# Agricultural-Robotics-Bonn/pagnerf

Hardware: NVIDIA B200
Metric: train rays/s (march+encode+decode+composite+backward) (higher is better)
Workload: dtype fp16 operands / f32 accumulate (decoders, tcgen05) + f32 (encoders, compositing) = the reference's autocast

## Files before the change

pagnerf_b200/csrc/decoder_tc.cu:

```cuda
#include "decoder_tc_common.cuh"

#define DC_THREADS 512
#define DC_NCG 4
#define DC_MAXK 4

struct DcTcLayout {
    int INP, nXc;
    int oG3, oGy, oOnesA, oX, oHd, oOnesB, oCin, oH1, oOnesC, oH2, oWd1, oWd2, oWc1, oWc2, oWc3, oBias, oPF, oDX, oXI, total;
};
__host__ __device__ inline DcTcLayout dc_tc_layout(int IN, bool bwd, bool img = false) {
    DcTcLayout l;
    l.INP = (IN + 15) & ~15;
    l.nXc = l.INP / 8;
    int o = 0;
    l.oG3 = o; o += bwd ? 2 * TCH : 0;
    l.oGy = o; o += bwd ? 2 * TCH : 0;
    l.oOnesA = o; o += bwd ? 2 * TCH : 0;
    l.oX = o; o += 8 * TCH;
    l.oHd = o; o += 8 * TCH;
    l.oOnesB = o; o += bwd ? 2 * TCH : 0;
    l.oCin = o; o += bwd ? 6 * TCH : 0;
    l.oH1 = o; o += bwd ? 8 * TCH : 0;
    l.oOnesC = o; o += bwd ? 2 * TCH : 0;
    l.oH2 = o; o += bwd ? 8 * TCH : 0;
// ... 149 lines not shown
        if (warp == 0 && elect_one()) { tc_fence_after(); mma16_fwd(tm + 64, aT1, wc2, 64, 64, 64, false); mb.commit(); }
        mb.wait();
        epi_relu16(tl + 64 + c16, bias + 144 + c16, T0 + 2 * cg * TCH, row);
        sync_to_mma();
        if (warp == 0 && elect_one()) { tc_fence_after(); mma16_fwd(tm, aT0, wc3, 16, 16, 64, false); mb.commit(); }
        mb.wait();
        if (cg == 0) {
            float c[16];
            tmem_ld16(tl, c);
            if (valid) {
#pragma unroll
                for (int j = 0; j < 3; ++j) rgb[3 * m + j] = 1.f / (1.f + __expf(-(c[j] + bias[208 + j])));
            }
        }
        tc_fence_before();
        __syncthreads();
    }
    tc_fence_before();
    __syncthreads();
    if (warp == 0) tmem_dealloc(tm, 128);
}

#define DCB_S0 0
#define DCB_S1 64
#define DCB_DWD1 128
#define DCB_DWD2 208
#define DCB_DWC1 288
#define DCB_DWC2 352
#define DCB_DWC3 432

struct DcWsLayout { int oWd1, oWd2, oWc1, oWc2, oWc3, total; };
__host__ __device__ inline DcWsLayout dc_ws_layout(int IN) {
    DcWsLayout w;
    int o = 0;
    w.oWd1 = o; o += 64 * IN;
    w.oWd2 = o; o += 16 * 64;
    w.oWc1 = o; o += (64 * CIN + 3) & ~3;
    w.oWc2 = o; o += 64 * 64;
    w.oWc3 = o; o += 3 * 64;
    w.total = o;
    return w;
}

template <bool IMG>
__global__ void __maxnreg__(96) dc_tc_bwd_kernel(const float* __restrict__ feats, const float* __restrict__ lodw,
                                                               const float* __restrict__ ray_d, int S, int64_t M, int IN,
                                                               DcParams p, const float* __restrict__ g_sigma,
                                                               const float* __restrict__ g_rgb, const float* __restrict__ scale_ptr,
                                                               float* __restrict__ g_feats, float* __restrict__ g_dir,
                                                               const int64_t* __restrict__ m_dev, const int64_t* __restrict__ ridx,
                                                               const uint4* __restrict__ pe16, float* __restrict__ ws) {
    if (m_dev) M = min(M, __ldg(m_dev));
    extern __shared__ __align__(128) uint8_t sm[];
    __shared__ uint64_t bar_s;
    __shared__ uint64_t xbar_s[2];
    __shared__ uint32_t tmem_s;
    __shared__ float gdir_s[2][128][3];
    const DcTcLayout l = dc_tc_layout(IN, true, IMG);
    const int tid = threadIdx.x, warp = warp_id_uniform(), lane = tid & 31;
    const int q = warp & 3, cg = warp >> 2, row = 32 * q + lane, c16 = 16 * cg;
    dc_tc_stage(sm, l, p, IN, lodw);
    for (int i = tid; i < 3 * 2 * TCH / 16; i += DC_THREADS) {
        const int t = i / (2 * TCH / 16), j = i - t * (2 * TCH / 16);
        uint4 u = make_uint4(0u, 0u, 0u, 0u);
        if (j < TCH / 16) u.x = 0x00003C00u;
        reinterpret_cast<uint4*>(sm + (t == 0 ? l.oOnesA : (t == 1 ? l.oOnesB : l.oOnesC)))[j] = u;
        if (IMG && t < 2) reinterpret_cast<uint4*>(sm + l.oXI + t * (2 + l.nXc) * TCH)[j] = u;
    }
    if (tid == 0) { mbar_init(&bar_s, 1); mbar_init(&xbar_s[0], 1); mbar_init(&xbar_s[1], 1); fence_mbar_init(); }
    if (warp == 0) tmem_alloc(&tmem_s, 512);
    sync_to_mma();
    tc_fence_after();
    const uint32_t tm = tmem_s, tl = tm + ((uint32_t)(q * 32) << 16);
    MmaBar mb{&bar_s, 0};
    const float* bias = reinterpret_cast<const float*>(sm + l.oBias);
    uint8_t *G3 = sm + l.oG3, *Gy = sm + l.oGy, *X = sm + l.oX, *Cin = sm + l.oCin, *Hd = sm + l.oHd, *H1 = sm + l.oH1, *H2 = sm + l.oH2;
    const uint32_t aG3 = smem_u32(G3), aGy = smem_u32(Gy), aX = smem_u32(X), aCin = smem_u32(Cin), aHd = smem_u32(Hd),
                   aH1 = smem_u32(H1), aH2 = smem_u32(H2), aOnesA = smem_u32(sm + l.oOnesA), aOnesB = smem_u32(sm + l.oOnesB),
                   aOnesC = smem_u32(sm + l.oOnesC);
    const uint32_t wd1 = smem_u32(sm + l.oWd1), wd2 = smem_u32(sm + l.oWd2), wc1 = smem_u32(sm + l.oWc1),
                   wc2 = smem_u32(sm + l.oWc2), wc3 = smem_u32(sm + l.oWc3);
    float4* pf = reinterpret_cast<float4*>(sm + l.oPF);
    const float scale = scale_ptr ? __ldg(scale_ptr) : 1.f;
    const float inv_scale = 1.f / scale;
    const bool do_rgb = g_rgb != nullptr;
    const int64_t ntiles = (M + 127) / 128;
    const uint32_t xbytes = (uint32_t)l.nXc * TCH, xstride = (uint32_t)(2 + l.nXc) * TCH;
    const uint8_t* fimg = reinterpret_cast<const uint8_t*>(feats);
    uint32_t xpar = 0;
    int xb = 0;
    if (IMG) {
        if ((int64_t)blockIdx.x < ntiles && warp == 0 && elect_one()) {
            mbar_expect_tx(&xbar_s[0], xbytes);
            bulk_g2s(sm + l.oXI + 2 * TCH, fimg + (size_t)blockIdx.x * xbytes, xbytes, &xbar_s[0]);
        }
    } else {
        if ((int64_t)blockIdx.x < ntiles) xpfc_issue<DC_MAXK>(pf, feats, nullptr, IN, (int64_t)blockIdx.x * 128, M);
        cp_async_wait_all();
    }
    __syncthreads();
    bool first = true;
    float* dxs = reinterpret_cast<float*>(sm + l.oDX);
    int64_t dx_tile = -1;
    for (int64_t tile = blockIdx.x; tile < ntiles; tile += gridDim.x, first = false, xb ^= 1) {
        const int64_t m = tile * 128 + row;
        const bool valid = m < M;
        const int64_t mm = valid ? m : M - 1;
        const uint32_t aXt = IMG ? smem_u32(sm + l.oXI + xb * xstride + 2 * TCH) : aX;
        const uint32_t aOnesXt = IMG ? smem_u32(sm + l.oXI + xb * xstride) : aOnesA;
        if (IMG) {
            if (g_feats && dx_tile >= 0 && warp == 0 && elect_one()) bulk_wait_read_all();
            if (tile + gridDim.x < ntiles && warp == 0 && elect_one()) {
                mbar_expect_tx(&xbar_s[xb ^ 1], xbytes);
                bulk_g2s(sm + l.oXI + (xb ^ 1) * xstride + 2 * TCH, fimg + (size_t)(tile + gridDim.x) * xbytes, xbytes, &xbar_s[xb ^ 1]);
            }
            mbar_wait(&xbar_s[xb], (xpar >> xb) & 1u);
            xpar ^= 1u << xb;
        } else {
            if (g_feats && dx_tile >= 0) dx_copy_out(dxs, g_feats, IN, dx_tile * 128, M);
            xpfc_consume<DC_NCG, DC_MAXK>(pf, false, IN, l.INP, X, row, cg);
        }
        float gs_row = 0.f, gr0 = 0.f, gr1 = 0.f, gr2 = 0.f;
        uint4 pa = make_uint4(0u, 0u, 0u, 0u), pb = pa;
        int64_t r = 0;
        if (cg == 0) {
            if (g_sigma && valid) gs_row = __ldg(g_sigma + m);
            if (do_rgb && valid) { gr0 = __ldg(g_rgb + 3 * m); gr1 = __ldg(g_rgb + 3 * m + 1); gr2 = __ldg(g_rgb + 3 * m + 2); }
        } else if (do_rgb && cg <= 2) {
            r = ridx ? ridx[mm] : mm / S;
            if (pe16) { pa = __ldg(pe16 + r * 4 + 2 * (cg - 1)); pb = __ldg(pe16 + r * 4 + 2 * (cg - 1) + 1); }
        }
        sync_to_mma();
        if (warp == 0 && elect_one()) { tc_fence_after(); mma16_fwd(tm + DCB_S0, aXt, wd1, 64, 64, l.INP, false); mb.commit(); }
        if (!IMG && tile + gridDim.x < ntiles)
            xpfc_issue<DC_MAXK>(pf, feats, nullptr, IN, (tile + gridDim.x) * 128, M);
        mb.wait();
        const uint32_t mask_d = epi_relu16(tl + DCB_S0 + c16, bias + c16, Hd + 2 * cg * TCH, row);
        sync_to_mma();
        if (warp == 0 && elect_one()) { tc_fence_after(); mma16_fwd(tm + DCB_S1, aHd, wd2, 16, 16, 64, false); mb.commit(); }
        mb.wait();
        bool y0pos = false;
        float vdir[3] = {0.f, 0.f, 0.f};
        uint32_t mask_1 = 0, mask_2 = 0;
        float dy[16];
#pragma unroll
        for (int i = 0; i < 16; ++i) dy[i] = 0.f;
        if (cg == 0) {
            float y[16];
            tmem_ld16(tl + DCB_S1, y);
#pragma unroll
            for (int i = 0; i < 16; ++i) y[i] += bias[64 + i];
            y0pos = y[0] > 0.f;
            if (do_rgb) { tile_store8(Cin, 0, row, y); tile_store8(Cin, 1, row, y + 8); }
        } else if (do_rgb && cg <= 2) {
            if (pe16 && !g_dir) stage_cin_pe16(Cin, row, cg, pa, pb);
            else {
                vdir[0] = -ray_d[3 * r]; vdir[1] = -ray_d[3 * r + 1]; vdir[2] = -ray_d[3 * r + 2];
                stage_cin_pe(Cin, row, cg, -vdir[0], -vdir[1], -vdir[2]);
            }
        }
        if (do_rgb) {
            sync_to_mma();
            if (warp == 0 && elect_one()) { tc_fence_after(); mma16_fwd(tm + DCB_S0, aCin, wc1, 64, 64, 48, false); mb.commit(); }
            mb.wait();
            mask_1 = epi_relu16(tl + DCB_S0 + c16, bias + 80 + c16, H1 + 2 * cg * TCH, row);
            sync_to_mma();
            if (warp == 0 && elect_one()) { tc_fence_after(); mma16_fwd(tm + DCB_S1, aH1, wc2, 64, 64, 64, false); mb.commit(); }
            mb.wait();
            mask_2 = epi_relu16(tl + DCB_S1 + c16, bias + 144 + c16, H2 + 2 * cg * TCH, row);
            sync_to_mma();
            if (warp == 0 && elect_one()) { tc_fence_after(); mma16_fwd(tm + DCB_S0, aH2, wc3, 16, 16, 64, false); mb.commit(); }
            mb.wait();
            if (cg == 0) {
                float c[16], g[16];
                tmem_ld16(tl + DCB_S0, c);
#pragma unroll
                for (int j = 0; j < 16; ++j) g[j] = 0.f;
                if (valid) {
                    const float gr[3] = {gr0, gr1, gr2};
#pragma unroll
                    for (int j = 0; j < 3; ++j) {
                        const float sg = 1.f / (1.f + __expf(-(c[j] + bias[208 + j])));
                        g[j] = gr[j] * sg * (1.f - sg) * scale;
                    }
                }
                tile_store8(G3, 0, row, g); tile_store8(G3, 1, row, g + 8);
            }
            sync_to_mma();
            if (warp == 0 && elect_one()) {
                tc_fence_after();
                mma16_bwd_weight(tm + DCB_DWC3, aG3, aOnesC, 80, !first);
                mma16_bwd_data(tm + DCB_S1, aG3, wc3, 64, 16, 16, false);
                mb.commit();
            }
            mb.wait();
            epi_grad16_nb(tl + DCB_S1 + c16, mask_2, H2 + 2 * cg * TCH, row);
            sync_to_mma();
            if (warp == 0 && elect_one()) {
                tc_fence_after();
                mma16_bwd_weight(tm + DCB_DWC2, aH2, aH1, 80, !first);
                mma16_bwd_data(tm + DCB_S0, aH2, wc2, 64, 64, 64, false);
                mb.commit();
            }
            mb.wait();
            epi_grad16_nb(tl + DCB_S0 + c16, mask_1, H1 + 2 * cg * TCH, row);
            sync_to_mma();
            if (warp == 0 && elect_one()) {
                tc_fence_after();
                mma16_bwd_weight(tm + DCB_DWC1, aH1, aOnesB, 64, !first);
                mma16_bwd_data(tm + DCB_S1, aH1, wc1, 48, 64, 64, false);
                mb.commit();
            }
            mb.wait();
            if (cg == 0) {
                tmem_ld16(tl + DCB_S1, dy);
            } else if (cg <= 2 && g_dir) {
                float g[16];
                tmem_ld16(tl + DCB_S1 + c16, g);
                float gv[3] = {0.f, 0.f, 0.f};
#pragma unroll
                for (int i = 0; i < 16; ++i) {
                    const int k = 16 * (cg - 1) + i;
                    if (k < 3) gv[k] += g[i];
                    else if (k < 3 + 3 * PE_F) { const int f = (k - 3) / 3, c = (k - 3) % 3; const float b = (float)(1 << f); gv[c] += b * cosf(vdir[c] * b) * g[i]; }
                    else if (k < PE_DIM) { const int f = (k - 3 - 3 * PE_F) / 3, c = (k - 3 - 3 * PE_F) % 3; const float b = (float)(1 << f); gv[c] -= b * sinf(vdir[c] * b) * g[i]; }
                }
                gdir_s[cg - 1][row][0] = gv[0]; gdir_s[cg - 1][row][1] = gv[1]; gdir_s[cg - 1][row][2] = gv[2];
            }
            if (g_dir) {
                __syncthreads();
                if (cg == 0 && valid) {
#pragma unroll
                    for (int c = 0; c < 3; ++c) g_dir[3 * m + c] = -(gdir_s[0][row][c] + gdir_s[1][row][c]) * inv_scale;
                }
            }
        } else if (g_dir && valid && cg == 0) {
            g_dir[3 * m] = 0.f; g_dir[3 * m + 1] = 0.f; g_dir[3 * m + 2] = 0.f;
        }
        if (cg == 0) {
            if (y0pos) dy[0] += gs_row * scale;
            if (!valid) {
#pragma unroll
                for (int i = 0; i < 16; ++i) dy[i] = 0.f;
            }
            tile_store8(Gy, 0, row, dy); tile_store8(Gy, 1, row, dy + 8);
        }
        sync_to_mma();
        if (warp == 0 && elect_one()) {
            tc_fence_after();
            mma16_bwd_weight(tm + DCB_DWD2, aGy, aHd, 80, !first);
            mma16_bwd_data(tm + DCB_S0, aGy, wd2, 64, 16, 16, false);
            mb.commit();
        }
        mb.wait();
        epi_grad16_nb(tl + DCB_S0 + c16, mask_d, Hd + 2 * cg * TCH, row);
        sync_to_mma();
        if (warp == 0 && elect_one()) {
            tc_fence_after();
            mma16_bwd_weight(tm + DCB_DWD1, aHd, aOnesXt, 16 + l.INP, !first);
            if (g_feats) mma16_bwd_data(tm + DCB_S1, aHd, wd1, l.INP, 64, 64, false);
            mb.commit();
        }
        mb.wait();
        if (IMG) {
            if (g_feats && c16 < l.INP) {
                float v[16];
                tmem_ld16(tl + DCB_S1 + c16, v);
                tile_store8(sm + l.oDX, 2 * cg, row, v);
                tile_store8(sm + l.oDX, 2 * cg + 1, row, v + 8);
                fence_async_smem();
            }
            dx_tile = tile;
            tc_fence_before();
            __syncthreads();
            if (g_feats && warp == 0 && elect_one()) bulk_s2g(reinterpret_cast<uint8_t*>(g_feats) + (size_t)tile * xbytes, sm + l.oDX, xbytes);
        } else {
            if (g_feats && c16 < l.INP) dx_stage16(tl + DCB_S1, dxs, row, IN, c16, inv_scale);
            dx_tile = tile;
            cp_async_wait_all();
            tc_fence_before();
            __syncthreads();
        }
    }
    if (IMG) {
        if (g_feats && dx_tile >= 0 && warp == 0 && elect_one()) bulk_wait_read_all();
    } else if (g_feats && dx_tile >= 0) dx_copy_out(dxs, g_feats, IN, dx_tile * 128, M);
    if (!first) {
        tc_fence_after();
        const bool plain = ws != nullptr;
        const DcWsLayout wl = dc_ws_layout(IN);
        float* wsb = plain ? ws + (size_t)blockIdx.x * wl.total : nullptr;
        float *dWd1 = plain ? wsb + wl.oWd1 : p.gWd1, *dWd2 = plain ? wsb + wl.oWd2 : p.gWd2, *dWc1 = plain ? wsb + wl.oWc1 : p.gWc1,
              *dWc2 = plain ? wsb + wl.oWc2 : p.gWc2, *dWc3 = plain ? wsb + wl.oWc3 : p.gWc3;
        if (c16 < l.INP) {
            float v[16];
            tmem_ld16(tl + DCB_DWD1 + 16 + c16, v);
            if (row < 64) {
#pragma unroll
                for (int i = 0; i < 16; ++i)
                    if (c16 + i < IN) {
                        const float x = v[i] * inv_scale * (lodw ? __ldg(lodw + c16 + i) : 1.f);
                        float* d = dWd1 + (size_t)row * IN + c16 + i;
                        if (plain) *d = x; else red_add_f32(d, x);
                    }
            }
        }
        flush_dw16(tl + DCB_DWD2, dWd2, row, 16, 64, c16, inv_scale, plain);
        if (do_rgb) {
            if (c16 < 48) flush_dw16(tl + DCB_DWC1 + 16, dWc1, row, 64, CIN, c16, inv_scale, plain);
            flush_dw16(tl + DCB_DWC2, dWc2, row, 64, 64, c16, inv_scale, plain);
            flush_dw16(tl + DCB_DWC3 + 16, dWc3, row, 3, 64, c16, inv_scale, plain);
        }
        if (cg == 0) {
            float v[16];
            tmem_ld16(tl + DCB_DWD1, v);
            if (row < 64) red_add_f32(p.gbd1 + row, v[0] * inv_scale);
            tmem_ld16(tl + DCB_DWD2 + 64, v);
            if (row < 16) red_add_f32(p.gbd2 + row, v[0] * inv_scale);
            if (do_rgb) {
                tmem_ld16(tl + DCB_DWC1, v);
                if (row < 64) red_add_f32(p.gbc1 + row, v[0] * inv_scale);
                tmem_ld16(tl + DCB_DWC2 + 64, v);
                if (row < 64) red_add_f32(p.gbc2 + row, v[0] * inv_scale);
                tmem_ld16(tl + DCB_DWC3, v);
                if (row < 3) red_add_f32(p.gbc3 + row, v[0] * inv_scale);
            }
        }
    }
    tc_fence_before();
    __syncthreads();
    if (warp == 0) tmem_dealloc(tm, 512);
// ... 491 lines not shown
```

pagnerf_b200/csrc/decoder_tc_common.cuh:

```cuda
#pragma once
#include "decoder_common.cuh"
#include "tc_common.cuh"
#include <cuda_fp16.h>

#define TCH TC_CHUNK_BYTES

#ifdef PAG_PHASE_TIMING
static __device__ unsigned long long pag_phase_clk[64];
#define PAG_PHASE_READER(name)                                                                        \
    extern "C" int name(unsigned long long* host64, int reset) {                                      \
        cudaError_t e = cudaMemcpyFromSymbol(host64, pag_phase_clk, sizeof(unsigned long long) * 64); \
        if (e != cudaSuccess) return (int)e;                                                          \
        if (reset) {                                                                                  \
            unsigned long long z[64] = {0};                                                           \
            e = cudaMemcpyToSymbol(pag_phase_clk, z, sizeof(z));                                      \
        }                                                                                             \
        return (int)e;                                                                                \
    }
#define PAG_PHASE_INIT()                                                     \
    __shared__ unsigned long long _ph_s[64];                                 \
    if (threadIdx.x < 64) _ph_s[threadIdx.x] = 0ull;                         \
    __syncthreads();                                                         \
    unsigned long long _ph_t = clock64()
#define PAG_PHASE(i)                                                         \
// ... 77 lines not shown
            const float send = hi ? v[i] : v[i + n];
            const float keep = hi ? v[i + n] : v[i];
            v[i] = keep + __shfl_xor_sync(0xffffffffu, send, o);
        }
    }
}
__device__ __forceinline__ int scatter_base(int lane, int n) {
    int f = 0, h = n / 2;
    for (int o = 16; o >= 1; o >>= 1, h >>= 1) f += (lane & o) ? h : 0;
    return f;
}
__device__ __forceinline__ void epi_grad64(uint32_t taddr, uint64_t mask, uint8_t* tile, int row, int lane, float (&dbacc)[2]) {
    float g[64];
#pragma unroll
    for (int c0 = 0; c0 < 64; c0 += 16) {
        float v[16];
        tmem_ld16(taddr + c0, v);
#pragma unroll
        for (int i = 0; i < 16; ++i) g[c0 + i] = ((mask >> (c0 + i)) & 1ull) ? v[i] : 0.f;
        tile_store8(tile, c0 / 8, row, g + c0);
        tile_store8(tile, c0 / 8 + 1, row, g + c0 + 8);
    }
    warp_reduce_scatter<64>(g, lane);
    dbacc[0] += g[0]; dbacc[1] += g[1];
}
__device__ __forceinline__ void grad16_store(float (&g)[16], uint8_t* tile, int row, int lane, float& dbacc) {
    tile_store8(tile, 0, row, g);
    tile_store8(tile, 1, row, g + 8);
#pragma unroll
    for (int o = 16, n = 8; o >= 2; o >>= 1, n >>= 1) {
        const bool hi = lane & o;
#pragma unroll
        for (int i = 0; i < n; ++i) {
            const float send = hi ? g[i] : g[i + n];
            const float keep = hi ? g[i + n] : g[i];
            g[i] = keep + __shfl_xor_sync(0xffffffffu, send, o);
        }
    }
    dbacc += g[0] + __shfl_xor_sync(0xffffffffu, g[0], 1);
}
__device__ __forceinline__ uint32_t epi_relu16(uint32_t taddr, const float* __restrict__ bias, uint8_t* tile2, int row) {
    float v[16];
    tmem_ld16(taddr, v);
    uint32_t mask = 0;
#pragma unroll
    for (int i = 0; i < 16; ++i) {
        v[i] = fmaxf(v[i] + bias[i], 0.f);
        mask |= (v[i] > 0.f) ? (1u << i) : 0u;
    }
    tile_store8(tile2, 0, row, v);
    tile_store8(tile2, 1, row, v + 8);
    return mask;
}
__device__ __forceinline__ void epi_grad16(uint32_t taddr, uint32_t mask, uint8_t* tile2, int row, int lane, float& dbacc) {
    float v[16];
    tmem_ld16(taddr, v);
#pragma unroll
    for (int i = 0; i < 16; ++i) v[i] = ((mask >> i) & 1u) ? v[i] : 0.f;
    grad16_store(v, tile2, row, lane, dbacc);
}
__device__ __forceinline__ void epi_grad16_nb(uint32_t taddr, uint32_t mask, uint8_t* tile2, int row) {
    float v[16];
    tmem_ld16(taddr, v);
#pragma unroll
    for (int i = 0; i < 16; ++i) v[i] = ((mask >> i) & 1u) ? v[i] : 0.f;
    tile_store8(tile2, 0, row, v);
    tile_store8(tile2, 1, row, v + 8);
}
struct WsSegs { int n; int off[6]; int len[6]; float* dst[6]; };
#define WS_GROUPS 16
static __global__ void __launch_bounds__(256) ws_reduce_kernel(const float* __restrict__ ws, int nblocks, int64_t M, const int64_t* __restrict__ m_dev,
                                                               int total, WsSegs segs) {
    if (m_dev) M = min(M, __ldg(m_dev));
    const int64_t ntiles = (M + 127) / 128;
    const int nact = (int)(ntiles < nblocks ? ntiles : nblocks);
    const int i = blockIdx.x * blockDim.x + threadIdx.x;
    if (i >= total) return;
    float* dst = nullptr;
#pragma unroll
    for (int s = 0; s < 6; ++s)
        if (s < segs.n && i >= segs.off[s] && i < segs.off[s] + segs.len[s] && segs.dst[s]) dst = segs.dst[s] + (i - segs.off[s]);
    if (!dst) return;
    float a0 = 0.f, a1 = 0.f;
    int b = blockIdx.y;
    for (; b + WS_GROUPS < nact; b += 2 * WS_GROUPS) { a0 += ws[(size_t)b * total + i]; a1 += ws[(size_t)(b + WS_GROUPS) * total + i]; }
    if (b < nact) a0 += ws[(size_t)b * total + i];
    if (blockIdx.y < nact) red_add_f32(dst, a0 + a1);
}

__device__ __forceinline__ void flush_dw16(uint32_t taddr, float* __restrict__ gW, int row, int OUT, int IN, int c0, float inv_scale,
                                           bool plain = false) {
    float v[16];
    tmem_ld16(taddr + c0, v);
    if (row < OUT) {
        float* dst = gW + (size_t)row * IN + c0;
        if (!(IN & 3) && !(reinterpret_cast<uintptr_t>(gW) & 15)) {
#pragma unroll
            for (int i = 0; i < 16; i += 4)
                if (c0 + i < IN) {
                    if (plain) *reinterpret_cast<float4*>(dst + i) = make_float4(v[i] * inv_scale, v[i + 1] * inv_scale, v[i + 2] * inv_scale, v[i + 3] * inv_scale);
                    else red_add_f32x4(dst + i, v[i] * inv_scale, v[i + 1] * inv_scale, v[i + 2] * inv_scale, v[i + 3] * inv_scale);
                }
        } else {
#pragma unroll
            for (int i = 0; i < 16; ++i)
                if (c0 + i < IN) {
                    if (plain) dst[i] = v[i] * inv_scale;
                    else red_add_f32(dst + i, v[i] * inv_scale);
                }
        }
    }
}

__device__ __forceinline__ void flush_dw(uint32_t taddr, float* __restrict__ gW, int row, int OUT, int IN, int ncols, float inv_scale) {
    for (int c0 = 0; c0 < ncols; c0 += 16) {
        float v[16];
        tmem_ld16(taddr + c0, v);
        if (row < OUT) {
// ... 214 lines not shown
```

pagnerf_b200/csrc/decoder_tc_fused.cu:

```cuda
#include "decoder_tc_common.cuh"

struct PanCompFwdLayout {
    int INP, nXc, CsP, CiP;
    int oX, oT1, oT2, oStage, oCR, oWs1, oWs2, oWi1, oWi2, oWi3, oBias, total;
};
__host__ __device__ inline PanCompFwdLayout pan_comp_fwd_layout(int IN, int Cs, int Ci) {
    PanCompFwdLayout l;
    l.INP = (IN + 15) & ~15; l.nXc = l.INP / 8;
    l.CsP = 16; l.CiP = Ci > 0 ? ((Ci + 15) & ~15) : 16;
    int o = 0;
    l.oX = o; o += l.nXc * TCH;
    l.oT1 = o; o += 8 * TCH;
    l.oT2 = o; o += 8 * TCH;
    l.oStage = 0;
    l.oCR = o; o += 4 * 32 * 8;
    o = (o + 15) & ~15;
    l.oWs1 = o; o += l.nXc * 64 * 16;
    l.oWs2 = o; o += 8 * l.CsP * 16;
    l.oWi1 = o; o += l.nXc * 64 * 16;
    l.oWi2 = o; o += 8 * 64 * 16;
    l.oWi3 = o; o += 8 * l.CiP * 16;
    l.oBias = o; o += (64 + l.CsP + 64 + 64 + l.CiP) * 4;
    l.total = o;
    return l;
// ... 203 lines not shown
#pragma unroll
                                for (int i = 0; i < 16; ++i) v[i] = fmaf(v[i], s2, bi3[c0 + 16 * h + i]);
                            }
#pragma unroll
                            for (int i = 0; i < 16; i += 2)
                                *reinterpret_cast<__half2*>(stage + lane * STG_LD + 16 * h + i) = __floats2half2_rn(v[i], v[i + 1]);
                        }
                    }
                    __syncwarp();
                    comp_block(stage, wc, wr, bmask, nrows, out_inst, Ci, c0, lane);
                    __syncwarp();
                }
            }
        }
        if (Cs > 0 && cg == 0) {
            float z[16];
            tmem_ld16(tl + semcol, z);
            float mx = -INFINITY, sum = 0.f;
#pragma unroll
            for (int j = 0; j < 16; ++j) { z[j] += bs2[j]; if (j < Cs) mx = fmaxf(mx, z[j]); }
#pragma unroll
            for (int j = 0; j < 16; ++j) { z[j] = (j < Cs) ? (sem_softmax ? __expf(z[j] - mx) : z[j]) : 0.f; sum += z[j]; }
            const float inv = sem_softmax ? 1.f / sum : 1.f;
#pragma unroll
            for (int j = 0; j < 16; ++j) stage[lane * STG_LD + j] = __float2half_rn(z[j] * inv);
            __syncwarp();
            comp_block(stage, wc, wr, bmask, nrows, out_sem, Cs, 0, lane);
            __syncwarp();
        }
        tc_fence_before();
        __syncthreads();
    }
    tc_fence_before();
    __syncthreads();
    if (warp == 0) tmem_dealloc(tm, 256);
}

#define PCB_S0 0
#define PCB_S1 64
#define PCB_SEMLOG 128
#define PCB_DW1J 208
#define PCB_DWS2T 256
#define PCB_DWI2 272
#define PCB_DWI3 352

#define PCB_THREADS 512
#define PCB_NCG 4
#define PCB_MAXK 3
#define PCB_NGC 16
#define PCB_SEM_CG 3

struct PanCompBwdLayout {
    int INP, nXc, CsP, CiP, nGi;
    int oGs, oX, oHs, oH1, oOnes, oH2, oGi, oW1, oWs2, oWi2, oWi3, oBias, oGC, oGSC, oPF, total;
};
__host__ __device__ inline PanCompBwdLayout pan_comp_bwd_layout(int IN, int Cs, int Ci, bool img = false) {
    PanCompBwdLayout l;
    l.INP = (IN + 15) & ~15; l.nXc = l.INP / 8;
    l.CsP = 16; l.CiP = Ci > 0 ? ((Ci + 15) & ~15) : 16; l.nGi = l.CiP / 8;
    int o = 0;
    l.oGs = o; o += 2 * TCH;
    l.oX = o; o += l.nXc * TCH;
    l.oHs = o; o += 8 * TCH;
    l.oH1 = o; o += 8 * TCH;
    l.oOnes = o; o += 2 * TCH;
    l.oH2 = o; o += 8 * TCH;
    l.oGi = o; o += l.nGi * TCH;
    l.oW1 = o; o += l.nXc * 128 * 16;
    l.oWs2 = o; o += 8 * l.CsP * 16;
    l.oWi2 = o; o += 8 * 64 * 16;
    l.oWi3 = o; o += 8 * l.CiP * 16;
    l.oBias = o; o += (64 + l.CsP + 64 + 64 + l.CiP) * 4;
    const int need = l.oGi + (l.nGi > 16 ? 32 : 16) * TCH;
    if (o < need) o = need;
    o = (o + 15) & ~15;
    l.oGC = o; o += PCB_NGC * l.CiP * 2;
    o = (o + 15) & ~15;
    l.oGSC = o; o += img ? PCB_NGC * 16 * 4 : 0;
    o = (o + 127) & ~127;
    l.oPF = o; o += img ? 2 * l.nXc * TCH : 2 * PCB_MAXK * PCB_THREADS * 16;
    l.total = o;
    return l;
}

struct PanWsLayout { int oWs1, oWs2, oWi1, oWi2, oWi3, total; };
__host__ __device__ inline PanWsLayout pan_ws_layout(int IN, int Cs, int Ci) {
    PanWsLayout w;
    int o = 0;
    w.oWs1 = o; o += 64 * IN;
    w.oWs2 = o; o += (Cs * 64 + 3) & ~3;
    w.oWi1 = o; o += 64 * IN;
    w.oWi2 = o; o += 64 * 64;
    w.oWi3 = o; o += (Ci * 64 + 3) & ~3;
    w.total = o;
    return w;
}
__device__ __forceinline__ void stage_w16_part(__half* img, const float* __restrict__ W, int OUT, int IN, int rows, int row0, int OUTP, int INP,
                                               const float* __restrict__ colscale) {
    const int n = (INP / 8) * rows * 8;
    for (int i = threadIdx.x; i < n; i += blockDim.x) {
        const int e = i & 7, r = (i >> 3) % rows, c = (i >> 3) / rows, in = c * 8 + e;
        float v = 0.f;
        if (W && r < OUT && in < IN) { v = __ldg(W + (size_t)r * IN + in); if (colscale) v *= __ldg(colscale + in); }
        img[((size_t)c * OUTP + row0 + r) * 8 + e] = __float2half_rn(v);
    }
}

__device__ __forceinline__ void load_g16(const __half* __restrict__ gc_row, const float* __restrict__ grow, int c0, int C, bool vec4,
                                         float scale, float (&g)[16]) {
    if (gc_row) {
        const uint4 a = *reinterpret_cast<const uint4*>(gc_row + c0), b = *reinterpret_cast<const uint4*>(gc_row + c0 + 8);
        const uint32_t u[8] = {a.x, a.y, a.z, a.w, b.x, b.y, b.z, b.w};
#pragma unroll
        for (int i = 0; i < 8; ++i) {
            const float2 f = __half22float2(*reinterpret_cast<const __half2*>(&u[i]));
            g[2 * i] = f.x; g[2 * i + 1] = f.y;
        }
    } else {
#pragma unroll
        for (int i = 0; i < 16; i += 4) {
            float4 t;
            if (vec4) t = (c0 + i < C) ? __ldg(reinterpret_cast<const float4*>(grow + c0 + i)) : make_float4(0.f, 0.f, 0.f, 0.f);
            else t = make_float4(c0 + i < C ? __ldg(grow + c0 + i) : 0.f, c0 + i + 1 < C ? __ldg(grow + c0 + i + 1) : 0.f,
                                 c0 + i + 2 < C ? __ldg(grow + c0 + i + 2) : 0.f, c0 + i + 3 < C ? __ldg(grow + c0 + i + 3) : 0.f);
            g[i] = __half2float(__float2half_rn(t.x * scale)); g[i + 1] = __half2float(__float2half_rn(t.y * scale));
            g[i + 2] = __half2float(__float2half_rn(t.z * scale)); g[i + 3] = __half2float(__float2half_rn(t.w * scale));
        }
    }
}

template <bool IMG>
__global__ void __launch_bounds__(PCB_THREADS) pan_comp_bwd_kernel(
    const float* __restrict__ feats, const float* __restrict__ dfeats, const float* __restrict__ lodw, int64_t M, int IN,
    PanParams p, int Cs, int Ci, int sem_softmax, int inst_softmax, float inst_inv_temp,
    const float* __restrict__ w, const float* __restrict__ alpha, const int64_t* __restrict__ ridx,
    const float* __restrict__ g_sem, const float* __restrict__ g_inst, int64_t R, const float* __restrict__ inst_lse,
    const float* __restrict__ scale_ptr, float* __restrict__ g_panop, const int64_t* __restrict__ m_dev, float* __restrict__ ws,
    float* __restrict__ gw_sem, float* __restrict__ gw_inst) {
    if (m_dev) M = min(M, __ldg(m_dev));
    extern __shared__ __align__(128) uint8_t sm[];
    __shared__ uint64_t bar_s;
    __shared__ uint64_t xbar_s;
    __shared__ uint32_t tmem_s;
    __shared__ float part_s[PCB_NCG][128];
    const PanCompBwdLayout l = pan_comp_bwd_layout(IN, Cs, Ci, IMG);
    const int tid = threadIdx.x, warp = warp_id_uniform(), lane = tid & 31;
    const int q = warp & 3, cg = warp >> 2;
    const int row = 32 * q + lane;
    const bool do_sem = (Cs > 0) && g_sem, do_inst = (Ci > 0) && g_inst;
    const float s2 = inst_softmax ? inst_inv_temp * LOG2E_F : inst_inv_temp;
    uint8_t *Gs = sm + l.oGs, *X = sm + l.oX, *Hs = sm + l.oHs, *H1 = sm + l.oH1, *H2 = sm + l.oH2, *Gi = sm + l.oGi;
    {
        float* b = reinterpret_cast<float*>(sm + l.oBias);
        __half* w1 = reinterpret_cast<__half*>(sm + l.oW1);
        stage_w16_part(w1, do_sem ? p.Ws1 : nullptr, 64, IN, 64, 0, 128, l.INP, lodw);
        stage_w16_part(w1, do_inst ? p.Wi1 : nullptr, 64, IN, 64, 64, 128, l.INP, lodw);
        if (do_sem) {
            stage_w16(reinterpret_cast<__half*>(sm + l.oWs2), p.Ws2, Cs, 64, l.CsP, 64);
            stage_b32(b, p.bs1, 64, 64); stage_b32(b + 64, p.bs2, Cs, l.CsP);
        }
        if (do_inst) {
            stage_w16(reinterpret_cast<__half*>(sm + l.oWi2), p.Wi2, 64, 64, 64, 64);
            stage_w16(reinterpret_cast<__half*>(sm + l.oWi3), p.Wi3, Ci, 64, l.CiP, 64);
            stage_b32(b + 64 + l.CsP, p.bi1, 64, 64); stage_b32(b + 128 + l.CsP, p.bi2, 64, 64);
            stage_bi3_scaled(b + 192 + l.CsP, p.bi3, Ci, l.CiP, s2, inst_softmax);
        }
        for (int i = tid; i < 2 * TCH / 16; i += PCB_THREADS) {
            uint4 u = make_uint4(0u, 0u, 0u, 0u);
            if (i < TCH / 16) u.x = 0x00003C00u;
            reinterpret_cast<uint4*>(sm + l.oOnes)[i] = u;
        }
        for (int i = tid; i < PCB_NGC * l.CiP / 8; i += PCB_THREADS)
            reinterpret_cast<uint4*>(sm + l.oGC)[i] = make_uint4(0u, 0u, 0u, 0u);
        if (!do_sem) for (int i = tid; i < 8 * TCH / 16; i += PCB_THREADS) reinterpret_cast<uint4*>(Hs)[i] = make_uint4(0u, 0u, 0u, 0u);
        if (!do_inst) for (int i = tid; i < 8 * TCH / 16; i += PCB_THREADS) reinterpret_cast<uint4*>(H1)[i] = make_uint4(0u, 0u, 0u, 0u);
    }
    if (tid == 0) { mbar_init(&bar_s, 1); mbar_init(&xbar_s, 1); fence_mbar_init(); }
    if (warp == 0) tmem_alloc(&tmem_s, 512);
    sync_to_mma();
    tc_fence_after();
    const uint32_t tm = tmem_s, tl = tm + ((uint32_t)(q * 32) << 16);
    MmaBar mb{&bar_s, 0};
    const float* bias = reinterpret_cast<const float*>(sm + l.oBias);
    const float *bs1 = bias, *bs2 = bias + 64, *bi1 = bias + 64 + l.CsP, *bi2 = bi1 + 64, *bi3 = bi2 + 64;
    const uint32_t aGs = smem_u32(Gs), aX = smem_u32(X), aHs = smem_u32(Hs), aH1 = smem_u32(H1), aH2 = smem_u32(H2), aGi = smem_u32(Gi),
                   aOnes = smem_u32(sm + l.oOnes);
    const uint32_t w1j = smem_u32(sm + l.oW1), ws2 = smem_u32(sm + l.oWs2), wi2 = smem_u32(sm + l.oWi2), wi3 = smem_u32(sm + l.oWi3);
    __half* gcache = reinterpret_cast<__half*>(sm + l.oGC);
    float* gsc = reinterpret_cast<float*>(sm + l.oGSC);
    const float scale = scale_ptr ? __ldg(scale_ptr) : 1.f;
    const float inv_scale = 1.f / scale;
    const int c16 = 16 * cg;
    const bool vec4 = !(Ci & 3);
    float db_s1 = 0.f, db_i1 = 0.f, db_s2 = 0.f;
    const int64_t ntiles = (M + 127) / 128;
    float4* pf = reinterpret_cast<float4*>(sm + l.oPF);
    int64_t n_ray = 0, n_ray0 = 0;
    float n_w = 0.f, n_lse = 0.f;
    const uint32_t xbytes = (uint32_t)l.nXc * TCH;
    uint8_t *XL = sm + l.oPF, *DL = sm + l.oPF + xbytes;
    const uint8_t *fimg = reinterpret_cast<const uint8_t*>(feats), *dimg = reinterpret_cast<const uint8_t*>(dfeats);
    uint32_t xpar = 0;
    if ((int64_t)blockIdx.x < ntiles) {
        const int64_t m0 = min((int64_t)blockIdx.x * 128 + row, M - 1);
        if (IMG) {
            if (warp == 0 && elect_one()) {
                mbar_expect_tx(&xbar_s, dimg ? 2 * xbytes : xbytes);
                bulk_g2s(XL, fimg + (size_t)blockIdx.x * xbytes, xbytes, &xbar_s);
                if (dimg) bulk_g2s(DL, dimg + (size_t)blockIdx.x * xbytes, xbytes, &xbar_s);
            }
        } else {
            xpfc_issue<PCB_MAXK>(pf, feats, dfeats, IN, (int64_t)blockIdx.x * 128, M);
        }
        n_ray = ridx[m0]; n_w = __ldg(w + m0); n_ray0 = ridx[(int64_t)blockIdx.x * 128];
        if (inst_lse) n_lse = __ldg(inst_lse + m0);
    }
    const int ci1 = Ci > 0 ? Ci : 1;
    const int gc_r0 = tid / ci1, gc_c0 = tid % ci1, gc_dr = PCB_THREADS / ci1, gc_dc = PCB_THREADS % ci1;
    bool first = true;
    float* dxs = reinterpret_cast<float*>(Hs);
    int64_t dx_tile = -1;
    PAG_PHASE_INIT();
    if (!IMG) cp_async_wait_all();
    __syncthreads();
    for (int64_t tile = blockIdx.x; tile < ntiles; tile += gridDim.x, first = false) {
        const int64_t m = tile * 128 + row;
        const bool valid = m < M;
        const int64_t mm = valid ? m : M - 1;
        const int64_t ray = n_ray, ray0 = n_ray0;
        const float w_row = n_w, lse_row = n_lse;
        const float a_row = __ldg(alpha + ray);
        if (IMG) {
            if (g_panop && dx_tile >= 0 && warp == 0 && elect_one()) bulk_wait_read_all();
            PAG_PHASE(0);
            mbar_wait(&xbar_s, xpar);
            xpar ^= 1u;
            tile_add16(X, XL, dimg ? DL : nullptr, (int)xbytes);
        } else {
            if (g_panop && dx_tile >= 0) dx_copy_out(dxs, g_panop, IN, dx_tile * 128, M);
            PAG_PHASE(0);
            xpfc_consume<PCB_NCG, PCB_MAXK>(pf, dfeats != nullptr, IN, l.INP, X, row, cg);
        }
        PAG_PHASE(1);
        {
            const int64_t tn = tile + gridDim.x;
            if (tn < ntiles) {
                const int64_t mn = min(tn * 128 + row, M - 1);
                n_ray = ridx[mn]; n_w = __ldg(w + mn); n_ray0 = ridx[tn * 128];
                if (inst_lse) n_lse = __ldg(inst_lse + mn);
            }
        }
        sync_to_mma(); PAG_PHASE(2);
        if (warp == 0 && elect_one()) {
            tc_fence_after();
            mma16_fwd(tm + PCB_S0, aX, w1j, 128, 128, l.INP, false);
            mb.commit();
        }
        PAG_PHASE(17);
        if (tile + gridDim.x < ntiles) {
            if (IMG) {
                if (warp == 0 && elect_one()) {
                    mbar_expect_tx(&xbar_s, dimg ? 2 * xbytes : xbytes);
                    bulk_g2s(XL, fimg + (size_t)(tile + gridDim.x) * xbytes, xbytes, &xbar_s);
                    if (dimg) bulk_g2s(DL, dimg + (size_t)(tile + gridDim.x) * xbytes, xbytes, &xbar_s);
                }
            } else {
                xpfc_issue<PCB_MAXK>(pf, feats, dfeats, IN, (tile + gridDim.x) * 128, M);
            }
        }
        PAG_PHASE(18);
        float gpre[7], gspre = 0.f;
        const int ngc_elems = PCB_NGC * Ci;
        if (IMG && do_sem && tid < PCB_NGC * Cs) {
            const int64_t src = ray0 * Cs + tid;
            gspre = (src < R * Cs) ? __ldg(g_sem + src) : 0.f;
        }
        if (do_inst) {
#pragma unroll
            for (int k = 0; k < 7; ++k) {
                const int e = tid + PCB_THREADS * k;
                const int64_t src = ray0 * Ci + e;
                gpre[k] = (e < ngc_elems && src < R * Ci) ? __ldg(g_inst + src) : 0.f;
            }
        }
        PAG_PHASE(19);
        mb.wait(); PAG_PHASE(3);
        const float cs = valid ? a_row * w_row : 0.f;
        uint32_t mask_s = 0, mask_1 = 0, mask_2 = 0;
        if (do_sem) {
// ... 86 lines not shown
                part_s[cg][row] = dot;
                __syncthreads(); PAG_PHASE(8);
                dot = (part_s[0][row] + part_s[1][row]) + (part_s[2][row] + part_s[3][row]);
                if (gw_inst && cg == 0 && valid) gw_inst[m] = dot * inv_scale;
            }
            const float c2 = cs * inst_inv_temp;
#pragma unroll
            for (int k = 0; k < 4; ++k) {
                const int c0 = 16 * (cg + PCB_NCG * k);
                if (c0 < l.CiP) {
                    float v[16], g[16];
                    load_g16(gc_row, grow, c0, Ci, vec4, scale, g);
                    if (inst_softmax) {
                        tmem_ld16(tl + c0, v);
#pragma unroll
                        for (int i = 0; i < 16; ++i) v[i] = c2 * v[i] * (g[i] - dot);
                    } else {
#pragma unroll
                        for (int i = 0; i < 16; ++i) v[i] = c2 * g[i];
                    }
                    tile_store8(Gi + (c0 / 8) * TCH, 0, row, v);
                    tile_store8(Gi + (c0 / 8) * TCH, 1, row, v + 8);
                }
            }
        }
        sync_to_mma(); PAG_PHASE(9);
        if (warp == 0 && elect_one()) {
            tc_fence_after();
            if (do_inst) {
                mma16_bwd_weight(tm + PCB_DWI3, aGi, aOnes, 80, !first);
                if (l.CiP > 128) mma16_bwd_weight(tm + PCB_DWI3 + 80, aGi + 16 * TCH, aOnes, 80, !first);
                mma16_bwd_data(tm + PCB_S1, aGi, wi3, 64, l.CiP, l.CiP, false);
            }
            if (do_sem) {
                mma16_bwd_weight(tm + PCB_DWS2T, aHs, aGs, 16, !first);
                mma16_bwd_data(tm + PCB_S0, aGs, ws2, 64, l.CsP, l.CsP, false);
            }
            mb.commit();
        }
        mb.wait(); PAG_PHASE(10);
        if (do_inst) epi_grad16_nb(tl + PCB_S1 + c16, mask_2, H2 + 2 * cg * TCH, row);
        if (do_sem) epi_grad16(tl + PCB_S0 + c16, mask_s, Hs + 2 * cg * TCH, row, lane, db_s1);
        if (do_inst) {
            sync_to_mma(); PAG_PHASE(11);
            if (warp == 0 && elect_one()) {
                tc_fence_after();
                mma16_bwd_weight(tm + PCB_DWI2, aH2, aH1, 80, !first);
                mma16_bwd_data(tm + PCB_S1, aH2, wi2, 64, 64, 64, false);
                mb.commit();
            }
            mb.wait(); PAG_PHASE(12);
            epi_grad16(tl + PCB_S1 + c16, mask_1, H1 + 2 * cg * TCH, row, lane, db_i1);
        }
        sync_to_mma(); PAG_PHASE(13);
        if (warp == 0 && elect_one()) {
            tc_fence_after();
            mma16_bwd_weight(tm + PCB_DW1J, aHs, aX, l.INP, !first);
            if (g_panop) mma16_bwd_data(tm + PCB_S0, aHs, w1j, l.INP, 128, 128, false);
            mb.commit();
        }
        mb.wait(); PAG_PHASE(14);
        if (IMG) {
            if (g_panop && c16 < l.INP) {
                float v[16];
                tmem_ld16(tl + PCB_S0 + c16, v);
                tile_store8(Hs, 2 * cg, row, v);
                tile_store8(Hs, 2 * cg + 1, row, v + 8);
                fence_async_smem();
            }
            dx_tile = tile;
            tc_fence_before();
            __syncthreads(); PAG_PHASE(15);
            if (g_panop && warp == 0 && elect_one()) bulk_s2g(reinterpret_cast<uint8_t*>(g_panop) + (size_t)tile * xbytes, Hs, xbytes);
        } else {
            if (g_panop && c16 < l.INP) dx_stage16(tl + PCB_S0, dxs, row, IN, c16, inv_scale);
            dx_tile = tile;
            cp_async_wait_all();
            tc_fence_before();
            __syncthreads(); PAG_PHASE(15);
        }
    }
    if (IMG) {
        if (g_panop && dx_tile >= 0 && warp == 0 && elect_one()) bulk_wait_read_all();
    } else if (g_panop && dx_tile >= 0) dx_copy_out(dxs, g_panop, IN, dx_tile * 128, M);
    if (!first) {
        tc_fence_after();
        const int f1 = scatter_base(lane, 32) >> 1;
        const bool own = !(lane & 1);
        const bool plain = ws != nullptr;
        const PanWsLayout wl = pan_ws_layout(IN, Cs, Ci);
        float* wsb = plain ? ws + (size_t)blockIdx.x * wl.total : nullptr;
        float *dWs1 = plain ? wsb + wl.oWs1 : p.gWs1, *dWs2 = plain ? wsb + wl.oWs2 : p.gWs2, *dWi1 = plain ? wsb + wl.oWi1 : p.gWi1,
              *dWi2 = plain ? wsb + wl.oWi2 : p.gWi2, *dWi3 = plain ? wsb + wl.oWi3 : p.gWi3;
        if (c16 < l.INP) {
            float* gW1 = (row < 64) ? (do_sem ? dWs1 : nullptr) : (do_inst ? dWi1 : nullptr);
            float v[16];
            tmem_ld16(tl + PCB_DW1J + c16, v);
            if (gW1) {
#pragma unroll
                for (int i = 0; i < 16; ++i)
                    if (c16 + i < IN) {
                        const float x = v[i] * inv_scale * (lodw ? __ldg(lodw + c16 + i) : 1.f);
                        float* d = gW1 + (size_t)(row & 63) * IN + c16 + i;
                        if (plain) *d = x; else red_add_f32(d, x);
                    }
            }
        }
        if (do_sem) {
            if (cg == 0) {
                float v[16];
                tmem_ld16(tl + PCB_DWS2T, v);
                if (row < 64) {
#pragma unroll
                    for (int j = 0; j < 16; ++j)
                        if (j < Cs) { if (plain) dWs2[(size_t)j * 64 + row] = v[j] * inv_scale; else red_add_f32(dWs2 + (size_t)j * 64 + row, v[j] * inv_scale); }
                }
            }
            if (own) red_add_f32(p.gbs1 + c16 + f1, db_s1 * inv_scale);
            if (own && cg == PCB_SEM_CG && f1 < Cs) red_add_f32(p.gbs2 + f1, db_s2 * inv_scale);
        }
        if (do_inst) {
            flush_dw16(tl + PCB_DWI2, dWi2, row, 64, 64, c16, inv_scale, plain);
            flush_dw16(tl + PCB_DWI3 + 16, dWi3, row, Ci, 64, c16, inv_scale, plain);
            if (l.CiP > 128) flush_dw16(tl + PCB_DWI3 + 96, dWi3 + (size_t)128 * 64, row, Ci - 128, 64, c16, inv_scale, plain);
            if (own) red_add_f32(p.gbi1 + c16 + f1, db_i1 * inv_scale);
            if (cg == 0) {
                float v[16];
                tmem_ld16(tl + PCB_DWI2 + 64, v);
                if (row < 64) red_add_f32(p.gbi2 + row, v[0] * inv_scale);
                tmem_ld16(tl + PCB_DWI3, v);
                if (row < Ci) red_add_f32(p.gbi3 + row, v[0] * inv_scale);
                if (l.CiP > 128) {
                    tmem_ld16(tl + PCB_DWI3 + 80, v);
                    if (128 + row < Ci) red_add_f32(p.gbi3 + 128 + row, v[0] * inv_scale);
                }
            }
// ... 114 lines not shown
```

Before: 14.11 million.

## Split weight-gradient MMAs onto a second mbarrier to overlap with epilogues

In the tcgen05 decoder backward kernels, the weight-gradient MMA is now issued after the data-gradient MMA and committed to its own mbarrier. Threads can therefore read the data-gradient result from tensor memory while the weight-gradient MMA is still running, and only wait for it before overwriting the shared tiles it reads. The fused panoptic kernel also gets a dedicated shared-memory DX staging buffer for the bulk store, so the wait on that store moves later in the loop instead of sitting at the top. This costs an extra barrier, some added waits, and more shared memory, and getting the buffer-reuse ordering wrong would be a correctness risk.

```diff
diff --git a/pagnerf_b200/csrc/decoder_tc.cu b/pagnerf_b200/csrc/decoder_tc.cu
--- a/pagnerf_b200/csrc/decoder_tc.cu
+++ b/pagnerf_b200/csrc/decoder_tc.cu
@@ -225,7 +225,7 @@
                                                                const uint4* __restrict__ pe16, float* __restrict__ ws) {
     if (m_dev) M = min(M, __ldg(m_dev));
     extern __shared__ __align__(128) uint8_t sm[];
-    __shared__ uint64_t bar_s;
+    __shared__ uint64_t bar_s[2];
     __shared__ uint64_t xbar_s[2];
     __shared__ uint32_t tmem_s;
     __shared__ float gdir_s[2][128][3];
@@ -240,12 +240,12 @@
         reinterpret_cast<uint4*>(sm + (t == 0 ? l.oOnesA : (t == 1 ? l.oOnesB : l.oOnesC)))[j] = u;
         if (IMG && t < 2) reinterpret_cast<uint4*>(sm + l.oXI + t * (2 + l.nXc) * TCH)[j] = u;
     }
-    if (tid == 0) { mbar_init(&bar_s, 1); mbar_init(&xbar_s[0], 1); mbar_init(&xbar_s[1], 1); fence_mbar_init(); }
+    if (tid == 0) { mbar_init(&bar_s[0], 1); mbar_init(&bar_s[1], 1); mbar_init(&xbar_s[0], 1); mbar_init(&xbar_s[1], 1); fence_mbar_init(); }
     if (warp == 0) tmem_alloc(&tmem_s, 512);
     sync_to_mma();
     tc_fence_after();
     const uint32_t tm = tmem_s, tl = tm + ((uint32_t)(q * 32) << 16);
-    MmaBar mb{&bar_s, 0};
+    MmaBar mb{&bar_s[0], 0}, mw{&bar_s[1], 0};
     const float* bias = reinterpret_cast<const float*>(sm + l.oBias);
     uint8_t *G3 = sm + l.oG3, *Gy = sm + l.oGy, *X = sm + l.oX, *Cin = sm + l.oCin, *Hd = sm + l.oHd, *H1 = sm + l.oH1, *H2 = sm + l.oH2;
     const uint32_t aG3 = smem_u32(G3), aGy = smem_u32(Gy), aX = smem_u32(X), aCin = smem_u32(Cin), aHd = smem_u32(Hd),
@@ -282,7 +282,6 @@
         const uint32_t aXt = IMG ? smem_u32(sm + l.oXI + xb * xstride + 2 * TCH) : aX;
         const uint32_t aOnesXt = IMG ? smem_u32(sm + l.oXI + xb * xstride) : aOnesA;
         if (IMG) {
-            if (g_feats && dx_tile >= 0 && warp == 0 && elect_one()) bulk_wait_read_all();
             if (tile + gridDim.x < ntiles && warp == 0 && elect_one()) {
                 mbar_expect_tx(&xbar_s[xb ^ 1], xbytes);
                 bulk_g2s(sm + l.oXI + (xb ^ 1) * xstride + 2 * TCH, fimg + (size_t)(tile + gridDim.x) * xbytes, xbytes, &xbar_s[xb ^ 1]);
@@ -362,27 +361,34 @@
             sync_to_mma();
             if (warp == 0 && elect_one()) {
                 tc_fence_after();
-                mma16_bwd_weight(tm + DCB_DWC3, aG3, aOnesC, 80, !first);
                 mma16_bwd_data(tm + DCB_S1, aG3, wc3, 64, 16, 16, false);
                 mb.commit();
+                mma16_bwd_weight(tm + DCB_DWC3, aG3, aOnesC, 80, !first);
+                mw.commit();
             }
             mb.wait();
-            epi_grad16_nb(tl + DCB_S1 + c16, mask_2, H2 + 2 * cg * TCH, row);
+            float g[16];
+            ld_grad16(tl + DCB_S1 + c16, mask_2, g);
+            mw.wait();
+            tile_store8(H2 + 2 * cg * TCH, 0, row, g); tile_store8(H2 + 2 * cg * TCH, 1, row, g + 8);
             sync_to_mma();
             if (warp == 0 && elect_one()) {
                 tc_fence_after();
-                mma16_bwd_weight(tm + DCB_DWC2, aH2, aH1, 80, !first);
                 mma16_bwd_data(tm + DCB_S0, aH2, wc2, 64, 64, 64, false);
                 mb.commit();
+                mma16_bwd_weight(tm + DCB_DWC2, aH2, aH1, 80, !first);
+                mw.commit();
             }
             mb.wait();
-            epi_grad16_nb(tl + DCB_S0 + c16, mask_1, H1 + 2 * cg * TCH, row);
+            ld_grad16(tl + DCB_S0 + c16, mask_1, g);
+            mw.wait();
+            tile_store8(H1 + 2 * cg * TCH, 0, row, g); tile_store8(H1 + 2 * cg * TCH, 1, row, g + 8);
             sync_to_mma();
             if (warp == 0 && elect_one()) {
                 tc_fence_after();
-                mma16_bwd_weight(tm + DCB_DWC1, aH1, aOnesB, 64, !first);
                 mma16_bwd_data(tm + DCB_S1, aH1, wc1, 48, 64, 64, false);
                 mb.commit();
+                mma16_bwd_weight(tm + DCB_DWC1, aH1, aOnesB, 64, !first);
             }
             mb.wait();
             if (cg == 0) {
@@ -421,18 +427,26 @@
         sync_to_mma();
         if (warp == 0 && elect_one()) {
             tc_fence_after();
-            mma16_bwd_weight(tm + DCB_DWD2, aGy, aHd, 80, !first);
             mma16_bwd_data(tm + DCB_S0, aGy, wd2, 64, 16, 16, false);
             mb.commit();
-        }
-        mb.wait();
-        epi_grad16_nb(tl + DCB_S0 + c16, mask_d, Hd + 2 * cg * TCH, row);
+            mma16_bwd_weight(tm + DCB_DWD2, aGy, aHd, 80, !first);
+            mw.commit();
+        }
+        mb.wait();
+        {
+            float g[16];
+            ld_grad16(tl + DCB_S0 + c16, mask_d, g);
+            mw.wait();
+            tile_store8(Hd + 2 * cg * TCH, 0, row, g); tile_store8(Hd + 2 * cg * TCH, 1, row, g + 8);
+        }
+        if (IMG && g_feats && dx_tile >= 0 && warp == 0 && elect_one()) bulk_wait_read_all();
         sync_to_mma();
         if (warp == 0 && elect_one()) {
             tc_fence_after();
-            mma16_bwd_weight(tm + DCB_DWD1, aHd, aOnesXt, 16 + l.INP, !first);
             if (g_feats) mma16_bwd_data(tm + DCB_S1, aHd, wd1, l.INP, 64, 64, false);
             mb.commit();
+            mma16_bwd_weight(tm + DCB_DWD1, aHd, aOnesXt, 16 + l.INP, !first);
+            mw.commit();
         }
         mb.wait();
         if (IMG) {
@@ -444,12 +458,14 @@
                 fence_async_smem();
             }
             dx_tile = tile;
+            mw.wait();
             tc_fence_before();
             __syncthreads();
             if (g_feats && warp == 0 && elect_one()) bulk_s2g(reinterpret_cast<uint8_t*>(g_feats) + (size_t)tile * xbytes, sm + l.oDX, xbytes);
         } else {
             if (g_feats && c16 < l.INP) dx_stage16(tl + DCB_S1, dxs, row, IN, c16, inv_scale);
             dx_tile = tile;
+            mw.wait();
             cp_async_wait_all();
             tc_fence_before();
             __syncthreads();
diff --git a/pagnerf_b200/csrc/decoder_tc_common.cuh b/pagnerf_b200/csrc/decoder_tc_common.cuh
--- a/pagnerf_b200/csrc/decoder_tc_common.cuh
+++ b/pagnerf_b200/csrc/decoder_tc_common.cuh
@@ -153,18 +153,19 @@
     tile_store8(tile2, 1, row, v + 8);
     return mask;
 }
+__device__ __forceinline__ void ld_grad16(uint32_t taddr, uint32_t mask, float (&v)[16]) {
+    tmem_ld16(taddr, v);
+#pragma unroll
+    for (int i = 0; i < 16; ++i) v[i] = ((mask >> i) & 1u) ? v[i] : 0.f;
+}
 __device__ __forceinline__ void epi_grad16(uint32_t taddr, uint32_t mask, uint8_t* tile2, int row, int lane, float& dbacc) {
     float v[16];
-    tmem_ld16(taddr, v);
-#pragma unroll
-    for (int i = 0; i < 16; ++i) v[i] = ((mask >> i) & 1u) ? v[i] : 0.f;
+    ld_grad16(taddr, mask, v);
     grad16_store(v, tile2, row, lane, dbacc);
 }
 __device__ __forceinline__ void epi_grad16_nb(uint32_t taddr, uint32_t mask, uint8_t* tile2, int row) {
     float v[16];
-    tmem_ld16(taddr, v);
-#pragma unroll
-    for (int i = 0; i < 16; ++i) v[i] = ((mask >> i) & 1u) ? v[i] : 0.f;
+    ld_grad16(taddr, mask, v);
     tile_store8(tile2, 0, row, v);
     tile_store8(tile2, 1, row, v + 8);
 }
diff --git a/pagnerf_b200/csrc/decoder_tc_fused.cu b/pagnerf_b200/csrc/decoder_tc_fused.cu
--- a/pagnerf_b200/csrc/decoder_tc_fused.cu
+++ b/pagnerf_b200/csrc/decoder_tc_fused.cu
@@ -279,7 +279,7 @@
 
 struct PanCompBwdLayout {
     int INP, nXc, CsP, CiP, nGi;
-    int oGs, oX, oHs, oH1, oOnes, oH2, oGi, oW1, oWs2, oWi2, oWi3, oBias, oGC, oGSC, oPF, total;
+    int oGs, oX, oHs, oH1, oOnes, oH2, oGi, oW1, oWs2, oWi2, oWi3, oBias, oGC, oGSC, oPF, oDX, total;
 };
 __host__ __device__ inline PanCompBwdLayout pan_comp_bwd_layout(int IN, int Cs, int Ci, bool img = false) {
     PanCompBwdLayout l;
@@ -306,6 +306,7 @@
     l.oGSC = o; o += img ? PCB_NGC * 16 * 4 : 0;
     o = (o + 127) & ~127;
     l.oPF = o; o += img ? 2 * l.nXc * TCH : 2 * PCB_MAXK * PCB_THREADS * 16;
+    l.oDX = o; o += img ? l.nXc * TCH : 0;
     l.total = o;
     return l;
 }
@@ -366,7 +367,7 @@
     float* __restrict__ gw_sem, float* __restrict__ gw_inst) {
     if (m_dev) M = min(M, __ldg(m_dev));
     extern __shared__ __align__(128) uint8_t sm[];
-    __shared__ uint64_t bar_s;
+    __shared__ uint64_t bar_s[2];
     __shared__ uint64_t xbar_s;
     __shared__ uint32_t tmem_s;
     __shared__ float part_s[PCB_NCG][128];
@@ -402,12 +403,12 @@
         if (!do_sem) for (int i = tid; i < 8 * TCH / 16; i += PCB_THREADS) reinterpret_cast<uint4*>(Hs)[i] = make_uint4(0u, 0u, 0u, 0u);
         if (!do_inst) for (int i = tid; i < 8 * TCH / 16; i += PCB_THREADS) reinterpret_cast<uint4*>(H1)[i] = make_uint4(0u, 0u, 0u, 0u);
     }
-    if (tid == 0) { mbar_init(&bar_s, 1); mbar_init(&xbar_s, 1); fence_mbar_init(); }
+    if (tid == 0) { mbar_init(&bar_s[0], 1); mbar_init(&bar_s[1], 1); mbar_init(&xbar_s, 1); fence_mbar_init(); }
     if (warp == 0) tmem_alloc(&tmem_s, 512);
     sync_to_mma();
     tc_fence_after();
     const uint32_t tm = tmem_s, tl = tm + ((uint32_t)(q * 32) << 16);
-    MmaBar mb{&bar_s, 0};
+    MmaBar mb{&bar_s[0], 0}, mw{&bar_s[1], 0};
     const float* bias = reinterpret_cast<const float*>(sm + l.oBias);
     const float *bs1 = bias, *bs2 = bias + 64, *bi1 = bias + 64 + l.CsP, *bi2 = bi1 + 64, *bi3 = bi2 + 64;
     const uint32_t aGs = smem_u32(Gs), aX = smem_u32(X), aHs = smem_u32(Hs), aH1 = smem_u32(H1), aH2 = smem_u32(H2), aGi = smem_u32(Gi),
@@ -458,10 +459,10 @@
         const float w_row = n_w, lse_row = n_lse;
         const float a_row = __ldg(alpha + ray);
         if (IMG) {
-            if (g_panop && dx_tile >= 0 && warp == 0 && elect_one()) bulk_wait_read_all();
             PAG_PHASE(0);
             mbar_wait(&xbar_s, xpar);
             xpar ^= 1u;
+            if (!first) mw.wait();
             tile_add16(X, XL, dimg ? DL : nullptr, (int)xbytes);
         } else {
             if (g_panop && dx_tile >= 0) dx_copy_out(dxs, g_panop, IN, dx_tile * 128, M);
@@ -654,27 +655,31 @@
             mb.wait(); PAG_PHASE(12);
             epi_grad16(tl + PCB_S1 + c16, mask_1, H1 + 2 * cg * TCH, row, lane, db_i1);
         }
+        if (IMG && g_panop && dx_tile >= 0 && warp == 0 && elect_one()) bulk_wait_read_all();
         sync_to_mma(); PAG_PHASE(13);
         if (warp == 0 && elect_one()) {
             tc_fence_after();
-            mma16_bwd_weight(tm + PCB_DW1J, aHs, aX, l.INP, !first);
             if (g_panop) mma16_bwd_data(tm + PCB_S0, aHs, w1j, l.INP, 128, 128, false);
             mb.commit();
+            mma16_bwd_weight(tm + PCB_DW1J, aHs, aX, l.INP, !first);
+            mw.commit();
         }
         mb.wait(); PAG_PHASE(14);
         if (IMG) {
+            uint8_t* DX = sm + l.oDX;
             if (g_panop && c16 < l.INP) {
                 float v[16];
                 tmem_ld16(tl + PCB_S0 + c16, v);
-                tile_store8(Hs, 2 * cg, row, v);
-                tile_store8(Hs, 2 * cg + 1, row, v + 8);
+                tile_store8(DX, 2 * cg, row, v);
+                tile_store8(DX, 2 * cg + 1, row, v + 8);
                 fence_async_smem();
             }
             dx_tile = tile;
             tc_fence_before();
             __syncthreads(); PAG_PHASE(15);
-            if (g_panop && warp == 0 && elect_one()) bulk_s2g(reinterpret_cast<uint8_t*>(g_panop) + (size_t)tile * xbytes, Hs, xbytes);
+            if (g_panop && warp == 0 && elect_one()) bulk_s2g(reinterpret_cast<uint8_t*>(g_panop) + (size_t)tile * xbytes, DX, xbytes);
         } else {
+            mw.wait();
             if (g_panop && c16 < l.INP) dx_stage16(tl + PCB_S0, dxs, row, IN, c16, inv_scale);
             dx_tile = tile;
             cp_async_wait_all();
@@ -684,6 +689,7 @@
     }
     if (IMG) {
         if (g_panop && dx_tile >= 0 && warp == 0 && elect_one()) bulk_wait_read_all();
+        if (!first) mw.wait();
     } else if (g_panop && dx_tile >= 0) dx_copy_out(dxs, g_panop, IN, dx_tile * 128, M);
     if (!first) {
         tc_fence_after();
```

After: 14.18 million (median of 6 runs). Within noise of the previous version (+0.5%).
